# JuanDuGit/DH3D

Hardware: AMD Instinct MI355X
Metric: point-clouds/sec (higher is better)
Workload: dtype f32; 1 GPU; local-descriptor forward (basic_config), N=8192 K=8, batch=8; clouds_per_gpu=8, clouds_total=8, points=8192, knn=8, parallelism=clouds sharded over 1 GPU(s), no data-path collective, weights=random-init (no checkpoint blobs exist upstream), steps_in_flight=4

## Files before the change

### dh3d_amd/csrc/knn.hip

```cpp
#include <float.h>
#include <limits.h>

#include <type_traits>

#include "cell_walk.h"
#include "common.h"
#include "keys.h"
#include "wave_ops.h"

#pragma clang fp contract(off)

namespace {

typedef float f32x2 __attribute__((ext_vector_type(2)));
typedef unsigned long long u64;

constexpr int kQueriesPerBlock = 256;
constexpr int kChunk = 1024;
constexpr int kQueue = 16;

struct KnnLadder {
  int log2ct;
  int ctmask;
  int cv;
// ... 215 lines not shown
                                                                    int32_t *__restrict__ nn,
                                                                    float *__restrict__ dist, const int *__restrict__ gate) {
  if (gate && !gate[(size_t)blockIdx.y * kCellInts + kCellFlag]) return;
  __shared__ __attribute__((aligned(16))) float s_c[kSortedWaves][64 * 3];
  __shared__ uint2 s_q[kSortedWaves][kQueue * 64];
  __shared__ int s_id[kSortedWaves][64];
  const int b = blockIdx.y;
  const int lane = threadIdx.x & 63, wave = threadIdx.x >> 6;
  const int NG = (N + 63) / 64;
  const int g = blockIdx.x * kSortedWaves + wave;
  if (g >= NG) return;
  const float4 *sc = sorted + (size_t)b * N;
  const float4 *gb = reinterpret_cast<const float4 *>(gbox) + (size_t)b * NG * 2;
  float *my_c = s_c[wave];
  uint2 *my_q = s_q[wave];
  int *my_id = s_id[wave];

  const int qi = g * 64 + lane;
  const bool valid = qi < N;
  const float4 pad = make_float4(INFINITY, INFINITY, INFINITY, __int_as_float(-1));
  float4 qr = valid ? sc[qi] : pad;
  const f32x2 qx2 = {qr.x, qr.x}, qy2 = {qr.y, qr.y}, qz2 = {qr.z, qr.z};
  const float4 qlo = gb[g * 2], qhi = gb[g * 2 + 1];

  KnnState<KMAX> st;
#pragma unroll
  for (int i = 0; i < KMAX; ++i) st.keys[i] = ~0ull;
  st.bound = INFINITY;
  int cnt = 0;
  float wave_bound = INFINITY;

  auto drain = [&]() {
    const int deepest = -wave_min_i32(-cnt);
    uint2 nxt = my_q[lane];
#pragma unroll 1
    for (int i = 0; i < deepest; ++i) {
      const uint2 e = nxt;
      if (i + 1 < deepest) nxt = my_q[(i + 1) * 64 + lane];
      if (i < cnt) knn_offer<KMAX>(st, __uint_as_float(e.x), (int)e.y, lad);
    }
    cnt = 0;
    wave_bound = wave_max_f32(valid ? st.bound : 0.f);
  };

  auto scan_group = [&](int gcc, const float4 cr) {
    my_c[cand4_slot(lane, 0)] = cr.x;
    my_c[cand4_slot(lane, 1)] = cr.y;
    my_c[cand4_slot(lane, 2)] = cr.z;
    my_id[lane] = __float_as_int(cr.w);
    __builtin_amdgcn_wave_barrier();
    const int clen = min(64, N - gcc * 64);
    for (int j = 0; j < clen; j += 32) {
      f32x2 s[4][4];
      float mn[4];
#pragma unroll
      for (int u = 0; u < 4; ++u) {
        knn_dist8(my_c + ((j >> 2) + 2 * u) * 12, qx2, qy2, qz2, s[u]);
        mn[u] = knn_min8(s[u]);
      }
      const float m = fminf(fminf(mn[0], mn[1]), fminf(mn[2], mn[3]));
      if (__any(valid && m <= st.bound)) {
#pragma unroll
        for (int u = 0; u < 4; ++u) {
          if (valid && mn[u] <= st.bound) {
#pragma unroll
            for (int t = 0; t < 8; ++t) {
              const float sv = s[u][t >> 1][t & 1];
              if (sv <= st.bound && j + 8 * u + t < clen) {
                my_q[cnt * 64 + lane] = make_uint2(__float_as_uint(sv), (unsigned)my_id[j + 8 * u + t]);
                ++cnt;
              }
            }
          }
          if (__any(cnt > kQueue - 8)) drain();
        }
      }
    }
    __builtin_amdgcn_wave_barrier();
  };
  auto load_group = [&](int gcc) { const int ci = gcc * 64 + lane; return ci < N ? sc[ci] : pad; };

  scan_group(g, qr);
  if (__any(cnt > 0)) drain();

  const int cg = g >> 6, NC = (NG + 63) >> 6;
  for (int tier = 0; tier < 2; ++tier) {
    for (int k = 0; k < 2 * NC; ++k) {
      const int ci = cg + ((k & 1) ? (k + 1) / 2 : -(k / 2));
      if (ci < 0 || ci >= NC) continue;
      const int c0 = ci * 64, gl = min(max(g - c0, 0), 63);
      const int gi = c0 + lane;
      const bool other = gi < NG && gi != g;
      float bd = INFINITY;
      float4 clo = make_float4(INFINITY, INFINITY, INFINITY, 0.f), chi = clo;
      if (other) {
        clo = gb[gi * 2];
        chi = gb[gi * 2 + 1];
        const float ex = fmaxf(fmaxf(clo.x - qhi.x, qlo.x - chi.x), 0.f);
        const float ey = fmaxf(fmaxf(clo.y - qhi.y, qlo.y - chi.y), 0.f);
        const float ez = fmaxf(fmaxf(clo.z - qhi.z, qlo.z - chi.z), 0.f);
        bd = (ex * ex + ey * ey + ez * ez) * 0.99999f;
      }
      unsigned long long mask =
          tier == 0 ? __ballot(other && bd == 0.f) : __ballot(other && bd > 0.f && bd <= wave_bound);
      if (!mask) continue;
      int l = knn_pick_near(mask, gl);
      mask &= ~(1ull << l);
      float4 nxt = load_group(c0 + l);
      while (true) {
        const int lcur = l;
        const float4 cr = nxt;
        const bool more = mask != 0;
        if (more) {
          l = knn_pick_near(mask, gl);
          mask &= ~(1ull << l);
          nxt = load_group(c0 + l);
        }
        const float bdl = wave_bcast_f32(bd, lcur);
        if (bdl <= wave_bound) {
          const float lx = wave_bcast_f32(clo.x, lcur), ly = wave_bcast_f32(clo.y, lcur), lz = wave_bcast_f32(clo.z, lcur);
          const float hx = wave_bcast_f32(chi.x, lcur), hy = wave_bcast_f32(chi.y, lcur), hz = wave_bcast_f32(chi.z, lcur);
          const float px = fmaxf(fmaxf(lx - qr.x, qr.x - hx), 0.f);
          const float py = fmaxf(fmaxf(ly - qr.y, qr.y - hy), 0.f);
          const float pz = fmaxf(fmaxf(lz - qr.z, qr.z - hz), 0.f);
          const float pd = (px * px + py * py + pz * pz) * 0.99999f;
          if (__any(valid && pd <= st.bound)) scan_group(c0 + lcur, cr);
        }
        if (!more) break;
      }
    }
  }
  if (__any(cnt > 0)) drain();

  if (valid) {
    const int y = __float_as_int(qr.w);
    int32_t *o_nn = nn + ((size_t)b * N + y) * K;
    float *o_d = dist + ((size_t)b * N + y) * K;
#pragma unroll
    for (int i = 0; i < KMAX; ++i) {
      if (i < K) {
        const unsigned tb = (unsigned)st.keys[i];
        if (st.keys[i] == ~0ull) {
          o_nn[i] = -1;
          o_d[i] = FLT_MAX;
        } else {
          o_nn[i] = (int)(((tb % (unsigned)lad.cv) << lad.log2ct) + tb / (unsigned)lad.cv);
          o_d[i] = __uint_as_float((unsigned)(st.keys[i] >> 32));
        }
      }
    }
  }
}

template <int S>
__host__ __device__ constexpr int knn_split_lds_bytes() {
  return S * (64 * 3 * 4 + kQueue * 64 * 8 + 64 * 4 + 64 * 4 + 64 * 4);
}
template <int KMAX, int S>
__device__ __forceinline__ void knn_split_body(const float4 *__restrict__ sorted, const float *__restrict__ gbox, int N, int K,
                                               const KnnLadder lad, int32_t *__restrict__ nn, float *__restrict__ dist,
                                               const int b, const int g, unsigned char *lds, const int wave0 = 0) {
  static_assert(KMAX * 64 * sizeof(u64) <= kQueue * 64 * sizeof(uint2), "a K-list fits its wave's survivor queue");
  uint2 (*s_q)[kQueue * 64] = reinterpret_cast<uint2 (*)[kQueue * 64]>(lds);
  float (*s_c)[64 * 3] = reinterpret_cast<float (*)[64 * 3]>(lds + S * kQueue * 64 * 8);
  int (*s_id)[64] = reinterpret_cast<int (*)[64]>(lds + S * (kQueue * 64 * 8 + 64 * 3 * 4));
  float (*s_share)[64] = reinterpret_cast<float (*)[64]>(lds + S * (kQueue * 64 * 8 + 64 * 3 * 4 + 64 * 4));
  float (*s_kth)[64] = reinterpret_cast<float (*)[64]>(lds + S * (kQueue * 64 * 8 + 64 * 3 * 4 + 64 * 8));
  constexpr int R = (KMAX + S - 1) / S - 1;
  const int lane = threadIdx.x & 63;
  const int wave = __builtin_amdgcn_readfirstlane((int)(threadIdx.x >> 6) - wave0);
  const int NG = (N + 63) / 64;
  const float4 *sc = sorted + (size_t)b * N;
  const float4 *gb = reinterpret_cast<const float4 *>(gbox) + (size_t)b * NG * 2;
  float *my_c = s_c[wave];
  uint2 *my_q = s_q[wave];
  int *my_id = s_id[wave];

  const int qi = g * 64 + lane;
  const bool valid = qi < N;
  const float4 pad = make_float4(INFINITY, INFINITY, INFINITY, __int_as_float(-1));
  const float4 qr = valid ? sc[qi] : pad;
  const f32x2 qx2 = {qr.x, qr.x}, qy2 = {qr.y, qr.y}, qz2 = {qr.z, qr.z};
  const float4 qlo = gb[g * 2], qhi = gb[g * 2 + 1];

  KnnState<KMAX> st;
#pragma unroll
  for (int i = 0; i < KMAX; ++i) st.keys[i] = ~0ull;
  st.bound = INFINITY;
  int cnt = 0;
  float wave_bound = INFINITY;
  s_share[wave][lane] = INFINITY;
  s_kth[wave][lane] = INFINITY;
  __syncthreads();

  auto adopt = [&](float mx) {
    float mk = st.bound;
#pragma unroll
    for (int w = 1; w < S; ++w) {
      mx = fmaxf(mx, s_share[(wave + w) % S][lane]);
      mk = fminf(mk, s_kth[(wave + w) % S][lane]);
    }
    st.bound = fminf(mk, mx);
    wave_bound = wave_max_f32(valid ? st.bound : 0.f);
  };

  auto drain = [&]() {
    const int deepest = -wave_min_i32(-cnt);
    uint2 nxt = my_q[lane];
#pragma unroll 1
    for (int i = 0; i < deepest; ++i) {
      const uint2 e = nxt;
      if (i + 1 < deepest) nxt = my_q[(i + 1) * 64 + lane];
      if (i < cnt) knn_offer<KMAX, true>(st, __uint_as_float(e.x), (int)e.y, lad);
    }
    cnt = 0;
    const unsigned hb = (unsigned)(st.keys[R] >> 32);
    float mx = INFINITY;
    if (hb <= 0x7f800000u) {
      const float dr = __uint_as_float(hb);
      mx = __fmul_rn(__fmul_rn(dr, dr), 1.000001f);
    }
    s_share[wave][lane] = mx;
    const unsigned hk = (unsigned)(st.keys[KMAX - 1] >> 32);
    if (hk <= 0x7f800000u) {
      const float dk = __uint_as_float(hk);
      s_kth[wave][lane] = __fmul_rn(__fmul_rn(dk, dk), 1.000001f);
    }
    adopt(mx);
  };

  auto scan_group = [&](int gcc, const float4 cr) {
    my_c[cand4_slot(lane, 0)] = cr.x;
    my_c[cand4_slot(lane, 1)] = cr.y;
    my_c[cand4_slot(lane, 2)] = cr.z;
    my_id[lane] = __float_as_int(cr.w);
    __builtin_amdgcn_wave_barrier();
    const int clen = min(64, N - gcc * 64);
    for (int j = 0; j < clen; j += 32) {
      f32x2 sq[4][4];
      float mn[4];
#pragma unroll
      for (int u = 0; u < 4; ++u) {
        knn_dist8(my_c + ((j >> 2) + 2 * u) * 12, qx2, qy2, qz2, sq[u]);
        mn[u] = knn_min8(sq[u]);
      }
      const float m = fminf(fminf(mn[0], mn[1]), fminf(mn[2], mn[3]));
      if (__any(valid && m <= st.bound)) {
#pragma unroll
        for (int u = 0; u < 4; ++u) {
          if (valid && mn[u] <= st.bound) {
#pragma unroll
            for (int t = 0; t < 8; ++t) {
              const float sv = sq[u][t >> 1][t & 1];
              if (sv <= st.bound && j + 8 * u + t < clen) {
                my_q[cnt * 64 + lane] = make_uint2(__float_as_uint(sv), (unsigned)my_id[j + 8 * u + t]);
                ++cnt;
              }
            }
          }
          if (__any(cnt > kQueue - 8)) drain();
        }
      }
    }
    __builtin_amdgcn_wave_barrier();
  };
  auto load_group = [&](int gcc) { const int ci = gcc * 64 + lane; return ci < N ? sc[ci] : pad; };

  const int NO = (NG - wave + S - 1) / S, NCH = (NO + 63) >> 6;
  const int jg = g / S, cj = min(jg >> 6, max(NCH - 1, 0));
  bool other = false;
  float bd = INFINITY;
  float4 clo = make_float4(INFINITY, INFINITY, INFINITY, 0.f), chi = clo;
  auto fetch_boxes = [&](int ci) {
    const int j = ci * 64 + lane, gi = j * S + wave;
    other = j < NO && gi != g;
    if (other) {
      clo = gb[gi * 2];
      chi = gb[gi * 2 + 1];
    }
  };
  auto test_boxes = [&]() {
    bd = INFINITY;
    if (other) {
      const float ex = fmaxf(fmaxf(clo.x - qhi.x, qlo.x - chi.x), 0.f);
      const float ey = fmaxf(fmaxf(clo.y - qhi.y, qlo.y - chi.y), 0.f);
      const float ez = fmaxf(fmaxf(clo.z - qhi.z, qlo.z - chi.z), 0.f);
      bd = (ex * ex + ey * ey + ez * ez) * 0.99999f;
    }
  };
  if (NCH == 1) fetch_boxes(0);

  {
    my_c[cand4_slot(lane, 0)] = qr.x;
    my_c[cand4_slot(lane, 1)] = qr.y;
    my_c[cand4_slot(lane, 2)] = qr.z;
    my_id[lane] = __float_as_int(qr.w);
    __builtin_amdgcn_wave_barrier();
    const int clen = min(64, N - g * 64);
    for (int blk = wave; blk * 8 < clen; blk += S) {
      f32x2 sq[4];
      knn_dist8(my_c + 2 * blk * 12, qx2, qy2, qz2, sq);
      if (valid) {
#pragma unroll
        for (int t = 0; t < 8; ++t) {
          const float sv = sq[t >> 1][t & 1];
          if (sv <= st.bound && blk * 8 + t < clen) {
            my_q[cnt * 64 + lane] = make_uint2(__float_as_uint(sv), (unsigned)my_id[blk * 8 + t]);
            ++cnt;
          }
        }
      }
      if (__any(cnt > 0)) drain();
    }
    __builtin_amdgcn_wave_barrier();
    __syncthreads();
    adopt(s_share[wave][lane]);
  }
  for (int tier = 0; tier < 2; ++tier) {
    for (int k = 0; k < 2 * NCH; ++k) {
      const int ci = cj + ((k & 1) ? (k + 1) / 2 : -(k / 2));
      if (ci < 0 || ci >= NCH) continue;
      if (NCH > 1) fetch_boxes(ci);
      if (NCH > 1 || tier == 0) test_boxes();
      const int gl = min(max(jg - ci * 64, 0), 63);
      if (tier == 1) adopt(s_share[wave][lane]);
      unsigned long long mask =
          tier == 0 ? __ballot(other && bd == 0.f) : __ballot(other && bd > 0.f && bd <= wave_bound);
      if (!mask) continue;
      int l = knn_pick_near(mask, gl);
      mask &= ~(1ull << l);
      float4 nxt = load_group((ci * 64 + l) * S + wave);
      while (true) {
        const int lcur = l;
        const float4 cr = nxt;
        const bool more = mask != 0;
        if (more) {
          l = knn_pick_near(mask, gl);
          mask &= ~(1ull << l);
          nxt = load_group((ci * 64 + l) * S + wave);
        }
        const float bdl = wave_bcast_f32(bd, lcur);
        if (bdl <= wave_bound) {
          const float lx = wave_bcast_f32(clo.x, lcur), ly = wave_bcast_f32(clo.y, lcur), lz = wave_bcast_f32(clo.z, lcur);
          const float hx = wave_bcast_f32(chi.x, lcur), hy = wave_bcast_f32(chi.y, lcur), hz = wave_bcast_f32(chi.z, lcur);
          const float px = fmaxf(fmaxf(lx - qr.x, qr.x - hx), 0.f);
          const float py = fmaxf(fmaxf(ly - qr.y, qr.y - hy), 0.f);
          const float pz = fmaxf(fmaxf(lz - qr.z, qr.z - hz), 0.f);
          const float pd = (px * px + py * py + pz * pz) * 0.99999f;
          if (__any(valid && pd <= st.bound)) scan_group((ci * 64 + lcur) * S + wave, cr);
        }
        if (!more) break;
      }
    }
  }
  if (__any(cnt > 0)) drain();

  for (int step = S / 2; step >= 1; step >>= 1) {
    __syncthreads();
    if (wave >= step && wave < 2 * step) {
#pragma unroll
      for (int i = 0; i < KMAX; ++i)
        my_q[i * 64 + lane] = make_uint2((unsigned)st.keys[i], (unsigned)(st.keys[i] >> 32));
    }
    __syncthreads();
    if (wave < step) {
      const uint2 *oq = s_q[wave + step];
#pragma unroll
      for (int i = 0; i < KMAX; ++i) {
        const uint2 e = oq[i * 64 + lane];
        const u64 key = ((u64)e.y << 32) | e.x;
        if (key < st.keys[KMAX - 1]) {
          st.keys[KMAX - 1] = key;
#pragma unroll
          for (int t = KMAX - 1; t > 0; --t) {
            const u64 a = st.keys[t - 1], c = st.keys[t];
            const bool lt = c < a;
            st.keys[t - 1] = lt ? c : a;
            st.keys[t] = lt ? a : c;
          }
        }
      }
    }
  }

  if (wave == 0 && valid) {
    const int y = __float_as_int(qr.w);
    int32_t *o_nn = nn + ((size_t)b * N + y) * K;
    float *o_d = dist + ((size_t)b * N + y) * K;
#pragma unroll
    for (int i = 0; i < KMAX; ++i) {
      if (i < K) {
        const unsigned tb = (unsigned)st.keys[i];
        if (st.keys[i] == ~0ull) {
          o_nn[i] = -1;
          o_d[i] = FLT_MAX;
        } else {
          o_nn[i] = (int)(((tb % (unsigned)lad.cv) << lad.log2ct) + tb / (unsigned)lad.cv);
          o_d[i] = __uint_as_float((unsigned)(st.keys[i] >> 32));
        }
      }
    }
  }
}


template <int KMAX, int S>
__global__ __launch_bounds__(64 * S) void knn_split_kernel(const float4 *__restrict__ sorted,
                                                         const float *__restrict__ gbox, int N, int K,
                                                         KnnLadder lad, int32_t *__restrict__ nn,
                                                         float *__restrict__ dist, const int *__restrict__ gate) {
  if (gate && !gate[(size_t)blockIdx.y * kCellInts + kCellFlag]) return;
  __shared__ __attribute__((aligned(16))) unsigned char s_lds[knn_split_lds_bytes<S>()];
  const unsigned ng = (unsigned)((N + 63) / 64);
  knn_split_body<KMAX, S>(sorted, gbox, N, K, lad, nn, dist, blockIdx.y, (int)((blockIdx.x + 37u * blockIdx.y) % ng), s_lds);
}


template <int CPL>
__device__ __forceinline__ void knn_small_select_all(float (&s)[CPL], int N, int K, const KnnLadder &lad, int lane,
                                                     unsigned &my_hi, unsigned &my_lo) {
  int ln = lane;
  asm volatile("" : "+v"(ln));
  unsigned kd[CPL];
#pragma unroll
  for (int c = 0; c < CPL; ++c) kd[c] = ln + 64 * c < N ? __float_as_uint(sqrtf(s[c])) : 0xFFFFFFFFu;
  u64 need = 0;
  u64 m1 = ~0ull, m2 = ~0ull;
  bool more = false;
  auto rescan = [&]() {
    m1 = ~0ull; m2 = ~0ull;
    int cnt = 0;
    asm volatile("" : "+v"(ln));
#pragma unroll
    for (int c = 0; c < CPL; ++c) {
      const int j = ln + 64 * c;
      const unsigned tb = j < N ? (unsigned)((j & lad.ctmask) * lad.cv + (j >> lad.log2ct)) : 0xFFFFFFFFu;
      const u64 key = ((u64)kd[c] << 32) | tb;
      const bool ok = key >= need && key != ~0ull;
      const bool c1 = ok && key < m1, c2 = ok && key < m2;
      m2 = c1 ? m1 : (c2 ? key : m2);
      m1 = c1 ? key : m1;
      cnt += ok ? 1 : 0;
    }
    more = cnt > 2;
  };
  rescan();
  for (int r = 0; r < K; ++r) {
    const unsigned hi = wave_min_u32((unsigned)(m1 >> 32));
    const unsigned lo = wave_min_u32((unsigned)(m1 >> 32) == hi ? (unsigned)m1 : 0xFFFFFFFFu);
    if (lane == r) { my_hi = hi; my_lo = lo; }
    const u64 sel = ((u64)hi << 32) | lo;
    if (sel == ~0ull) break;
    need = sel + 1;
    const bool won = m1 == sel;
    const bool dry = won && m2 == ~0ull && more;
    m1 = won ? m2 : m1;
    m2 = won ? ~0ull : m2;
    if (__ballot(dry) != 0ull) rescan();
  }
}
// ... 120 lines not shown
    return dh3d_launch_status();                                                                                 \
  }
    DH3D_SMALL_CASE(8) DH3D_SMALL_CASE(16) DH3D_SMALL_CASE(32)
#undef DH3D_SMALL_CASE
    return DH3D_ERR_UNSUPPORTED;
  }
  dim3 grid(dh3d_cdiv(N, kQueriesPerBlock), B), block(kQueriesPerBlock);
#define DH3D_LANE_CASE(KM)                                                                                       \
  if (p.kmax == KM) {                                                                                            \
    hipLaunchKernelGGL((knn_kernel<KM, XYZ>), grid, block, 0, s, pos, N, K, lad, nn, dist);                      \
    return dh3d_launch_status();                                                                                 \
  }
  DH3D_LANE_CASE(4) DH3D_LANE_CASE(8) DH3D_LANE_CASE(16) DH3D_LANE_CASE(32) DH3D_LANE_CASE(64)
#undef DH3D_LANE_CASE
  return DH3D_ERR_UNSUPPORTED;
}

template <int KMAX>
__global__ __launch_bounds__(256) void knn_anydp_kernel(const float *__restrict__ pos, int Dp, int N, int K, KnnLadder lad,
                                                        int32_t *__restrict__ nn, float *__restrict__ dist) {
  __shared__ float s_c[16][256];
  const int b = blockIdx.y, y = blockIdx.x * 256 + threadIdx.x;
  const float *pc = pos + (size_t)b * Dp * N;
  float q[16];
#pragma unroll
  for (int dp = 0; dp < 16; ++dp) q[dp] = (dp < Dp && y < N) ? pc[(size_t)dp * N + y] : 0.f;
  u64 keys[KMAX];
#pragma unroll
  for (int i = 0; i < KMAX; ++i) keys[i] = ~0ull;
  for (int x0 = 0; x0 < N; x0 += 256) {
    __syncthreads();
    for (int dp = 0; dp < Dp; ++dp) s_c[dp][threadIdx.x] = x0 + (int)threadIdx.x < N ? pc[(size_t)dp * N + x0 + threadIdx.x] : 0.f;
    __syncthreads();
    const int cnt = min(256, N - x0);
    for (int j = 0; j < cnt; ++j) {
      float sum = 0.f;
      for (int dp = 0; dp < Dp; ++dp) {
        const float val = s_c[dp][j] - q[dp];
        sum = __builtin_fmaf(val, val, sum);
      }
      const float d = sqrtf(sum);
      const int x = x0 + j;
      const unsigned tb = (unsigned)((x & lad.ctmask) * lad.cv + (x >> lad.log2ct));
      const u64 key = ((u64)__float_as_uint(d) << 32) | tb;
      if (key < keys[K - 1]) {
        int i = K - 1;
        while (i > 0 && keys[i - 1] > key) { keys[i] = keys[i - 1]; --i; }
        keys[i] = key;
      }
    }
  }
  if (y >= N) return;
  int32_t *o_nn = nn + ((size_t)b * N + y) * K;
  float *o_d = dist + ((size_t)b * N + y) * K;
  for (int i = 0; i < K; ++i) {
    if (keys[i] == ~0ull) { o_nn[i] = -1; o_d[i] = 3.402823466e+38f; continue; }
    const unsigned tb = (unsigned)keys[i];
    o_nn[i] = (int)(((tb % (unsigned)lad.cv) << lad.log2ct) + tb / (unsigned)lad.cv);
    o_d[i] = __uint_as_float((unsigned)(keys[i] >> 32));
  }
}

}

DH3D_API int dh3d_knn_bruteforce(const float *positions, int B, int Dp, int N, int K, int32_t *nn,
                                 float *dist, void *stream) {
  DH3D_REQUIRE(positions && nn && dist && B > 0 && N > 0 && K > 0 && Dp > 0);
  DH3D_SUPPORTED(K <= kKnnMaxK && B <= kKnnMaxB);
  if (Dp == 3) return knn_launch<false>(positions, B, N, K, nn, dist, (hipStream_t)stream);
  DH3D_SUPPORTED(Dp <= kAnyDpMax);
  const KnnLadder lad = knn_ladder(N);
  dim3 grid(dh3d_cdiv(N, 256), B), block(256);
  hipStream_t s = (hipStream_t)stream;
  const int km = knn_anydp_width(K);
#define DH3D_ANYDP_CASE(KM)                                                                                      \
  if (km == KM) {                                                                                                \
    hipLaunchKernelGGL(knn_anydp_kernel<KM>, grid, block, 0, s, positions, Dp, N, K, lad, nn, dist);             \
    return dh3d_launch_status();                                                                                 \
  }
  DH3D_ANYDP_CASE(8) DH3D_ANYDP_CASE(16) DH3D_ANYDP_CASE(64)
#undef DH3D_ANYDP_CASE
  return DH3D_ERR_UNSUPPORTED;
}

DH3D_API int dh3d_knn_bruteforce_xyz(const float *xyz, int B, int N, int K, int32_t *nn, float *dist,
                                     void *stream) {
  DH3D_REQUIRE(xyz && nn && dist && B > 0 && N > 0 && K > 0);
  DH3D_SUPPORTED(K <= kKnnMaxK && B <= kKnnMaxB);
  return knn_launch<true>(xyz, B, N, K, nn, dist, (hipStream_t)stream);
}

DH3D_API int dh3d_knn_bruteforce_plan(int B, int Dp, int N, int K) {
  if (!(B > 0 && N > 0 && K > 0 && Dp > 0) || !(K <= kKnnMaxK && B <= kKnnMaxB)) return -1;
  if (Dp != 3) return Dp <= kAnyDpMax ? 3 * 65536 + knn_anydp_width(K) : -1;
  const KnnPlan p = knn_plan(B, N, K);
  return p.cpl > 0 ? 1 * 65536 + p.cpl * 256 + p.q : 2 * 65536 + p.kmax;
}

struct KnnSortedPlan {
  int s, kmax;
};
static KnnSortedPlan knn_sorted_plan(int B, int N, int K) {
  const long long groups = (long long)((N + 63) / 64) * B;
  KnnSortedPlan p{groups <= 256 ? 8 : groups <= 1280 ? 4 : groups <= 4096 ? 2 : 0, knn_list_width(K)};
  if (p.kmax > 16) p.s = 0;
  if (p.s == 8 && p.kmax == 4) p.kmax = 8;
  return p;
}

static int knn_sorted_launch(const float *sorted, const float *gbox, int B, int N, int K, int32_t *nn, float *dist,
                             const int *gate, void *stream) {
  DH3D_REQUIRE(sorted && gbox && nn && dist && B > 0 && N > 0 && K > 0);
  DH3D_SUPPORTED(K <= kKnnMaxK && B <= kKnnMaxB);
  const KnnLadder lad = knn_ladder(N);
  const int NG = (N + 63) / 64;
  dim3 grid(dh3d_cdiv(NG, kSortedWaves), B), block(64 * kSortedWaves);
  hipStream_t s = (hipStream_t)stream;
  const float4 *so = reinterpret_cast<const float4 *>(sorted);
  const KnnSortedPlan p = knn_sorted_plan(B, N, K);
  if (p.s > 0) {
    dim3 sgrid(NG, B);
#define DH3D_SPLIT_CASE(KM, SS)                                                                               \
  if (p.kmax == KM && p.s == SS) {                                                                           \
    hipLaunchKernelGGL((knn_split_kernel<KM, SS>), sgrid, dim3(64 * SS), 0, s, so, gbox, N, K, lad, nn, dist, gate); \
    return dh3d_launch_status();                                                                             \
  }
    DH3D_SPLIT_CASE(4, 2) DH3D_SPLIT_CASE(4, 4)
    DH3D_SPLIT_CASE(8, 2) DH3D_SPLIT_CASE(8, 4) DH3D_SPLIT_CASE(8, 8)
    DH3D_SPLIT_CASE(16, 2) DH3D_SPLIT_CASE(16, 4) DH3D_SPLIT_CASE(16, 8)
#undef DH3D_SPLIT_CASE
    return DH3D_ERR_UNSUPPORTED;
  }
#define DH3D_SORTED_CASE(KM)                                                                                  \
  if (p.kmax == KM) {                                                                                        \
    hipLaunchKernelGGL((knn_sorted_kernel<KM>), grid, block, 0, s, so, gbox, N, K, lad, nn, dist, gate);      \
    return dh3d_launch_status();                                                                             \
  }
  DH3D_SORTED_CASE(4) DH3D_SORTED_CASE(8) DH3D_SORTED_CASE(16) DH3D_SORTED_CASE(32) DH3D_SORTED_CASE(64)
#undef DH3D_SORTED_CASE
  return DH3D_ERR_UNSUPPORTED;
}

DH3D_API int dh3d_knn_sorted(const float *sorted, const float *gbox, int B, int N, int K, int32_t *nn,
                             float *dist, void *stream) {
  return knn_sorted_launch(sorted, gbox, B, N, K, nn, dist, nullptr, stream);
}

DH3D_API int dh3d_knn_sorted_plan(int B, int N, int K) {
  if (!(B > 0 && N > 0 && K > 0) || !(K <= kKnnMaxK && B <= kKnnMaxB)) return -1;
  const KnnSortedPlan p = knn_sorted_plan(B, N, K);
  return p.s * 256 + p.kmax;
}

constexpr int kGridCap = 256;
constexpr int kGridRow = kGridCap + 2;
constexpr int kGridScreenCap = 80;
static_assert(kGridScreenCap % 16 == 0 && kGridScreenCap * 6 <= kGridCap * 2, "the screened drain's row");

__device__ __forceinline__ unsigned knn_spread4(unsigned v) {
  return (v & 1u) | ((v & 2u) << 2) | ((v & 4u) << 4) | ((v & 8u) << 6);
}
__device__ __forceinline__ void knn_cswap(u64 &a, u64 &b) {
  const bool lt = b < a;
  const u64 lo = lt ? b : a, hi = lt ? a : b;
  a = lo; b = hi;
}
template <int CTRL>
__device__ __forceinline__ u64 knn_dpp_u64(u64 v) {
  const int lo = __builtin_amdgcn_update_dpp(0, (int)(unsigned)v, CTRL, 0xF, 0xF, true);
  const int hi = __builtin_amdgcn_update_dpp(0, (int)(unsigned)(v >> 32), CTRL, 0xF, 0xF, true);
  return ((u64)(unsigned)hi << 32) | (unsigned)lo;
}
template <int CTRL>
__device__ __forceinline__ int knn_dpp_i32(int v) {
  return __builtin_amdgcn_update_dpp(0, v, CTRL, 0xF, 0xF, true);
}
template <int CTRL>
__device__ __forceinline__ void knn_merge_step(KnnState<8> &st) {
  u64 c[8];
#pragma unroll
  for (int i = 0; i < 8; ++i) {
    const u64 mine = st.keys[i], theirs = knn_dpp_u64<CTRL>(st.keys[7 - i]);
    c[i] = mine < theirs ? mine : theirs;
  }
  knn_cswap(c[0], c[4]); knn_cswap(c[1], c[5]); knn_cswap(c[2], c[6]); knn_cswap(c[3], c[7]);
  knn_cswap(c[0], c[2]); knn_cswap(c[1], c[3]); knn_cswap(c[4], c[6]); knn_cswap(c[5], c[7]);
  knn_cswap(c[0], c[1]); knn_cswap(c[2], c[3]); knn_cswap(c[4], c[5]); knn_cswap(c[6], c[7]);
#pragma unroll
  for (int i = 0; i < 8; ++i) st.keys[i] = c[i];
}
__device__ __forceinline__ void knn_bound_of_list(KnnState<8> &st) {
  const unsigned hb = (unsigned)(st.keys[7] >> 32);
  if (hb <= 0x7f800000u) {
    const float dk = __uint_as_float(hb);
    st.bound = __fmul_rn(__fmul_rn(dk, dk), 1.000001f);
  }
}
template <int L>
__device__ __forceinline__ void knn_merge_sublanes(KnnState<8> &st) {
  if (L >= 2) knn_merge_step<0xB1>(st);
  if (L >= 4) knn_merge_step<0x4E>(st);
  if (L >= 8) knn_merge_step<0x141>(st);
  knn_bound_of_list(st);
}
template <int L>
__device__ __forceinline__ void knn_merge_after_sparse_pass(KnnState<8> &st, int sub) {
  if (L != 4 || __any(sub != 0 && st.keys[0] != ~0ull)) {
    knn_merge_sublanes<L>(st);
    return;
  }
#pragma unroll
  for (int i = 0; i < 8; ++i) st.keys[i] = knn_dpp_u64<0x00>(st.keys[i]);
  knn_bound_of_list(st);
}

template <int L, int SF>
__global__ __launch_bounds__(256) void knn_grid_kernel(const float4 *__restrict__ sorted, const float *__restrict__ gbox,
                                                      const int *__restrict__ cells, int N, int K, int D, KnnLadder lad,
                                                      int32_t *__restrict__ nn, float *__restrict__ dist) {
  constexpr int QB = 256 / L;
  static_assert(SF == 0 || (L == 4 && SF <= 4), "the merged scan: 64 queries per workgroup, at most four waves");
  constexpr int kGridLds = 3 * 64 * 4 + QB * kGridRow * 2 + QB * 4;
  constexpr int kSplitLds = SF == 2 ? 2 * knn_split_lds_bytes<2>() : SF > 0 ? knn_split_lds_bytes<(SF > 0 ? SF : 1)>() : 0;
  __shared__ __attribute__((aligned(16))) unsigned char s_raw[kGridLds > kSplitLds ? kGridLds : kSplitLds];
  const int b = blockIdx.y, lane = threadIdx.x & 63, sub = lane & (L - 1);
  if (cells[(size_t)b * kCellInts + kCellFlag]) {
    if constexpr (SF > 0) {
      const int ngq = (N + 63) / 64;
      if constexpr (SF == 2) {
        const int half = (int)(threadIdx.x >> 7), pairs = (ngq + 1) / 2;
        if ((int)blockIdx.x >= pairs) return;
        const int g0 = (int)blockIdx.x + half * pairs;
        if (g0 >= ngq) return;
        knn_split_body<8, 2>(sorted, gbox, N, K, lad, nn, dist, b, (int)(((unsigned)g0 + 37u * (unsigned)b) % (unsigned)ngq),
                             s_raw + half * knn_split_lds_bytes<2>(), half * 2);
      } else if (threadIdx.x < 64 * SF) {
        knn_split_body<8, (SF > 0 ? SF : 1)>(sorted, gbox, N, K, lad, nn, dist, b, (int)((blockIdx.x + 37u * (unsigned)b) % (unsigned)ngq), s_raw);
      }
    }
    return;
  }
  const int qi = (int)((blockIdx.x + 37u * (unsigned)b) % gridDim.x) * QB + threadIdx.x / L;
  const bool valid = qi < N;
  const float4 *sc = sorted + (size_t)b * N;
  const CellGrid g = cell_grid(cells, b);
  const int *ct = g.ct;
  const float lo[3] = {g.lo[0], g.lo[1], g.lo[2]}, scl[3] = {g.scl[0], g.scl[1], g.scl[2]};
  const int nb[3] = {g.nb[0], g.nb[1], g.nb[2]};
  const float4 qr = sc[valid ? qi : N - 1];
  const float q[3] = {qr.x, qr.y, qr.z};
  int nc[3], drop[3];
  sched_bits(g.sched, nc, kGridSteps - D);
#pragma unroll
  for (int a = 0; a < 3; ++a) drop[a] = nb[a] - nc[a];
  const int span = 1 << D;
  int cq[3], gmax[3];
  float w[3], eps[3];
#pragma unroll
  for (int a = 0; a < 3; ++a) {
    cq[a] = min((4 << nb[a]) - 1, max(0, (int)((q[a] - lo[a]) * scl[a]))) >> (2 + drop[a]);
    gmax[a] = ((1 << nb[a]) >> drop[a]) - 1;
    w[a] = (float)(4 << drop[a]) / scl[a];
    eps[a] = 2.5e-6f * ((float)(4 << nb[a]) / scl[a]);
  }
  unsigned (*s_ctab)[64] = reinterpret_cast<unsigned (*)[64]>(s_raw);
  cell_deposit_tables(g.sched, nc[0], nc[1], nc[2], kGridSteps - D, s_ctab);
  auto tab_code = [&](int ax, int ay, int az) { return s_ctab[0][ax & 63] | s_ctab[1][ay & 63] | s_ctab[2][az & 63]; };
  KnnState<8> st;
#pragma unroll
  for (int i = 0; i < 8; ++i) st.keys[i] = ~0ull;
  st.bound = valid ? INFINITY : -1.f;

  auto axis_d2 = [&](int a, int o) {
    const float l = lo[a] + (float)(cq[a] + o) * w[a];
    const float d = fmaxf(fmaxf(fmaxf(l - q[a], q[a] - (l + w[a])), 0.f) - eps[a], 0.f);
    return d * d;
  };
  float d2x[5];
  unsigned bitx[5];
  bool okx[5];
#pragma unroll
  for (int t = 0; t < 5; ++t) {
    const int ax = cq[0] + t - 2;
    okx[t] = (unsigned)ax <= (unsigned)gmax[0];
    d2x[t] = okx[t] ? axis_d2(0, t - 2) : INFINITY;
    bitx[t] = s_ctab[0][ax & 63];
  }
  auto inside = [&](int R) {
    float G = INFINITY;
#pragma unroll
    for (int a = 0; a < 3; ++a) {
      if (cq[a] - R > 0) G = fminf(G, (q[a] - (lo[a] + (float)(cq[a] - R) * w[a])) - eps[a]);
      if (cq[a] + R < gmax[a]) G = fminf(G, ((lo[a] + (float)(cq[a] + R + 1) * w[a]) - q[a]) - eps[a]);
    }
    if (G == INFINITY) return true;
    G = fmaxf(G, 0.f);
    return st.bound < G * G * 0.99999f;
  };

  auto keep_one_copy = [&]() {
    if (sub != 0) {
#pragma unroll
      for (int i = 0; i < 8; ++i) st.keys[i] = ~0ull;
    }
  };
  unsigned short (*s_list)[kGridRow] = reinterpret_cast<unsigned short (*)[kGridRow]>(s_raw + 3 * 64 * 4);
  int *s_cnt = reinterpret_cast<int *>(s_raw + 3 * 64 * 4 + QB * kGridRow * 2);
  const int qs = threadIdx.x / L;
  auto direct = [&](int j) {
    const float4 r = sc[j];
    const float dx = r.x - q[0], dy = r.y - q[1], dz = r.z - q[2];
    knn_offer<8, false>(st, fmaf(dz, dz, fmaf(dy, dy, dx * dx)), __float_as_int(r.w), lad);
  };
  auto enqueue = [&](int beg, int end) {
    const int len = end - beg;
    if (len <= 0) return;
    const int off = atomicAdd(&s_cnt[qs], len);
    const int fit = min(len, kGridCap - off);
    for (int k = 0; k < fit; ++k) s_list[qs][off + k] = (unsigned short)(beg + k);
    for (int k = max(fit, 0); k < len; ++k) direct(beg + k);
  };
  auto drain_screened = [&]() __attribute__((always_inline)) {
    const int T = s_cnt[qs];
    if constexpr (L != 4) return min(T, kGridCap);
    const bool screen = !__any(T > kGridScreenCap) && __any(T > 32);
    const int ns = screen ? T : 0;
    unsigned short *row = s_list[qs];
    float *s2v = reinterpret_cast<float *>(row + kGridScreenCap);
    float m1 = INFINITY, m2 = INFINITY;
#pragma unroll 1
    for (int k0 = 0; k0 < ns; k0 += 4 * L) {
      float4 r[4];
#pragma unroll
      for (int u = 0; u < 4; ++u) r[u] = sc[row[min(k0 + sub + u * L, ns - 1)]];
      wave_lds_sync();
#pragma unroll
      for (int u = 0; u < 4; ++u) {
        const int i = k0 + sub + u * L;
        const float dx = r[u].x - q[0], dy = r[u].y - q[1], dz = r[u].z - q[2];
        const float s = i < ns ? fmaf(dz, dz, fmaf(dy, dy, dx * dx)) : __builtin_nanf("");
        m2 = s < m1 ? m1 : fminf(m2, s);
        m1 = fminf(m1, s);
        s2v[i] = s;
        row[i] = (unsigned short)__float_as_int(r[u].w);
      }
    }
    float U = m2;
    U = fmaxf(U, __int_as_float(knn_dpp_i32<0xB1>(__float_as_int(U))));
    U = fmaxf(U, __int_as_float(knn_dpp_i32<0x4E>(__float_as_int(U))));
    const float thr = __fmul_rn(U, 1.000001f);
    wave_lds_sync();
    int c = 0;
#pragma unroll 1
    for (int k0 = 0; k0 < ns; k0 += 4 * L) {
      float s[4];
      unsigned short id[4];
#pragma unroll
      for (int u = 0; u < 4; ++u) {
        s[u] = s2v[k0 + sub + u * L];
        id[u] = row[k0 + sub + u * L];
      }
      wave_lds_sync();
      int n = 0, at[4];
#pragma unroll
      for (int u = 0; u < 4; ++u) {
        at[u] = n;
        n += s[u] <= thr ? 1 : 0;
      }
      const int n1 = knn_dpp_i32<0x90>(n);
      int p = n + (sub >= 1 ? n1 : 0);
      const int p2 = knn_dpp_i32<0x40>(p);
      p += sub >= 2 ? p2 : 0;
      const int first = c + p - n;
#pragma unroll
      for (int u = 0; u < 4; ++u)
        if (s[u] <= thr) {
          s2v[first + at[u]] = s[u];
          row[first + at[u]] = id[u];
        }
      c += knn_dpp_i32<0xFF>(p);
      wave_lds_sync();
    }
    float s_n = s2v[sub];
    int id_n = row[sub];
#pragma unroll 1
    for (int j = sub; j < c; j += L) {
      const float s = s_n;
      const int id = id_n;
      const int jn = min(j + L, kGridScreenCap - 1);
      s_n = s2v[jn];
      id_n = row[jn];
      knn_offer<8, false>(st, s, id, lad);
    }
    return screen ? 0 : min(T, kGridCap);
  };
  auto drain = [&](auto screen) __attribute__((always_inline)) {
    wave_lds_sync();
    int total;
    if constexpr (decltype(screen)::value) total = drain_screened();
    else total = min(s_cnt[qs], kGridCap);
#pragma unroll 1
    for (int base = sub; base < total; base += 4 * L) {
      float4 r[4];
      bool ok[4];
#pragma unroll
      for (int u = 0; u < 4; ++u) {
        const int i = base + u * L;
        ok[u] = i < total;
        r[u] = sc[s_list[qs][min(i, total - 1)]];
      }
#pragma unroll
      for (int u = 0; u < 4; ++u) {
        const float dx = r[u].x - q[0], dy = r[u].y - q[1], dz = r[u].z - q[2];
        const float s2 = fmaf(dz, dz, fmaf(dy, dy, dx * dx));
        knn_offer<8, false>(st, ok[u] ? s2 : __builtin_nanf(""), __float_as_int(r[u].w), lad);
      }
    }
    wave_lds_sync();
  };
  auto column = [&](auto tmask, int dy, int dz) __attribute__((always_inline)) {
    constexpr int TMASK = decltype(tmask)::value;
    const int ay = cq[1] + dy - 2, az = cq[2] + dz - 2;
    if ((unsigned)ay > (unsigned)gmax[1] || (unsigned)az > (unsigned)gmax[2]) return;
    const float d2yz = axis_d2(1, dy - 2) + axis_d2(2, dz - 2);
    const unsigned bityz = tab_code(0, ay, az);
    int beg[5], end[5];
#pragma unroll
    for (int t = 0; t < 5; ++t)
      if (TMASK >> t & 1) {
        beg[t] = ct[bityz | bitx[t]];
        end[t] = ct[(bityz | bitx[t]) + span];
      }
    if constexpr (TMASK != 0b01110) {
#pragma unroll
      for (int t = 0; t < 5; ++t)
        if (TMASK >> t & 1) {
          if (!okx[t] || (d2yz + d2x[t]) * 0.99999f > st.bound) continue;
          enqueue(beg[t], end[t]);
        }
    } else {
      int len[5], tot = 0;
#pragma unroll
      for (int t = 0; t < 5; ++t)
        if (TMASK >> t & 1) {
          len[t] = okx[t] && !((d2yz + d2x[t]) * 0.99999f > st.bound) ? end[t] - beg[t] : 0;
          tot += len[t];
        }
      if (tot == 0) return;
      int off = atomicAdd(&s_cnt[qs], tot);
#pragma unroll
      for (int t = 0; t < 5; ++t)
        if (TMASK >> t & 1) {
          const int fit = min(len[t], kGridCap - off);
          unsigned short *dst = &s_list[qs][off];
#pragma unroll
          for (int k = 0; k < 4; ++k)
            if (k < fit) dst[k] = (unsigned short)(beg[t] + k);
          for (int k = 4; k < fit; ++k) dst[k] = (unsigned short)(beg[t] + k);
          for (int k = max(fit, 0); k < len[t]; ++k) direct(beg[t] + k);
          off += len[t];
        }
    }
  };
  auto begin_pass = [&]() __attribute__((always_inline)) {
    if (sub == 0) s_cnt[qs] = 0;
    __builtin_amdgcn_fence(__ATOMIC_SEQ_CST, "wavefront");
    __builtin_amdgcn_wave_barrier();
  };
  begin_pass();
  if constexpr (L == 4) {
    const int ay = cq[1] + 1, az = cq[2] + 1;
    const bool mine = sub < 3 && (unsigned)ay <= (unsigned)gmax[1] && (unsigned)az <= (unsigned)gmax[2];
    const bool okc = sub == 0 ? okx[1] : sub == 1 ? okx[2] : okx[3];
    const float d2c = (sub == 0 ? d2x[1] : sub == 1 ? d2x[2] : d2x[3]) + axis_d2(1, 1) + axis_d2(2, 1);
    const unsigned code = tab_code(0, ay, az) | (sub == 0 ? bitx[1] : sub == 1 ? bitx[2] : bitx[3]);
    const int beg9 = ct[mine ? code : 0], end9 = ct[mine ? code + span : 0];
#pragma unroll 1
    for (int ci = sub; ci < 8; ci += L) column(std::integral_constant<int, 0b01110>{}, 1 + ci % 3, 1 + ci / 3);
    if (mine && okc && !(d2c * 0.99999f > st.bound)) enqueue(beg9, end9);
  } else {
#pragma unroll 1
    for (int ci = sub; ci < 9; ci += L) column(std::integral_constant<int, 0b01110>{}, 1 + ci % 3, 1 + ci / 3);
  }
  drain(std::true_type{});
  knn_merge_sublanes<L>(st);
  keep_one_copy();
  begin_pass();
  bool exact = false;
  int ylo = -2, zlo = -2, ny = 5, ncol = valid ? 25 : 0;
  if (valid && st.bound < INFINITY) {
    const float r = sqrtf(st.bound) * 1.0001f;
    int dlo[3], dhi[3];
#pragma unroll
    for (int a = 0; a < 3; ++a) {
      const float inv = scl[a] / (float)(4 << drop[a]);
      dlo[a] = min(0, max(0, (int)floorf((q[a] - r - eps[a] - lo[a]) * inv)) - cq[a]);
      dhi[a] = max(0, min(gmax[a], (int)floorf((q[a] + r + eps[a] - lo[a]) * inv)) - cq[a]);
    }
    const int by = dhi[1] - dlo[1] + 1, bc = by * (dhi[2] - dlo[2] + 1);
    if (dlo[0] >= -2 && dhi[0] <= 2 && bc <= 128) {
      exact = true;
      ylo = dlo[1]; zlo = dlo[2]; ny = by; ncol = bc;
    }
  }
#pragma unroll 1
  for (int ci = sub; ci < ncol; ci += L) {
    const int iz = ci / ny, dy = ylo + (ci - iz * ny), dz = zlo + iz;
    if (abs(dy) <= 1 && abs(dz) <= 1) column(std::integral_constant<int, 0b10001>{}, dy + 2, dz + 2);
    else column(std::integral_constant<int, 0b11111>{}, dy + 2, dz + 2);
  }
  drain(std::false_type{});
  knn_merge_after_sparse_pass<L>(st, sub);
  const bool done = !valid || exact || inside(2);
  if (__any(!done)) {
    if (done) {
      keep_one_copy();
    } else {
#pragma unroll
      for (int i = 0; i < 8; ++i) st.keys[i] = ~0ull;
      const int NG = (N + 63) >> 6;
      const float4 *gb = reinterpret_cast<const float4 *>(gbox) + (size_t)b * NG * 2;
#pragma unroll 1
      for (int g = sub; g < NG; g += L) {
        const float4 lo4 = gb[2 * g], hi4 = gb[2 * g + 1];
        const float ex = fmaxf(fmaxf(lo4.x - q[0], q[0] - hi4.x), 0.f), ey = fmaxf(fmaxf(lo4.y - q[1], q[1] - hi4.y), 0.f),
                    ez = fmaxf(fmaxf(lo4.z - q[2], q[2] - hi4.z), 0.f);
        if ((ex * ex + ey * ey + ez * ez) * 0.99999f > st.bound) continue;
        const int j1 = min(N, g * 64 + 64);
#pragma unroll 1
        for (int j = g * 64; j < j1; j += 8) {
          float4 r8[8];
#pragma unroll
          for (int u = 0; u < 8; ++u) r8[u] = sc[min(j + u, j1 - 1)];
#pragma unroll
          for (int u = 0; u < 8; ++u) {
            const float dx = r8[u].x - q[0], dy = r8[u].y - q[1], dz = r8[u].z - q[2];
            const float s2 = fmaf(dz, dz, fmaf(dy, dy, dx * dx));
            knn_offer<8, false>(st, j + u < j1 ? s2 : __builtin_nanf(""), __float_as_int(r8[u].w), lad);
          }
        }
      }
    }
    knn_merge_sublanes<L>(st);
  }
  if (valid) {
    const int y = __float_as_int(qr.w);
#pragma unroll
    for (int e = 0; e < 8 / L; ++e) {
      const int slot = e * L + sub;
      if (slot >= K) break;
      u64 key = st.keys[0];
#pragma unroll
      for (int i = 1; i < 8; ++i) key = slot == i ? st.keys[i] : key;
      const size_t o = ((size_t)b * N + y) * K + slot;
      if (key == ~0ull) {
        nn[o] = -1;
        dist[o] = FLT_MAX;
      } else {
        const unsigned tb = (unsigned)key;
        nn[o] = (int)(((tb % (unsigned)lad.cv) << lad.log2ct) + tb / (unsigned)lad.cv);
        dist[o] = __uint_as_float((unsigned)(key >> 32));
      }
    }
  }
}

constexpr int kGridLanes = 4;

struct KnnGridPlan {
  int sf, drop;
};
static KnnGridPlan knn_grid_plan(int B, int N) {
  KnnGridPlan p{0, 0};
  while (p.drop < 6 && ((long long)N << p.drop) <= 3072) ++p.drop;
  const long long groups = (long long)((N + 63) / 64) * B;
  if (kGridLanes == 4 && groups <= 4096) p.sf = groups > 1280 ? 2 : 4;
  return p;
}

DH3D_API int dh3d_knn_grid_plan(int B, int N, int K) {
  if (B <= 0 || N <= 0 || K <= 0 || K > 8 || N > 16384 || B > 65535) return -1;
  const KnnGridPlan p = knn_grid_plan(B, N);
  return p.sf + 16 * p.drop;
}

DH3D_API int dh3d_knn_grid(const float *sorted, const float *gbox, const int32_t *cells, int B, int N, int K, int32_t *nn,
                           float *dist, void *stream) {
  DH3D_REQUIRE(sorted && gbox && cells && nn && dist && B > 0 && N > 0 && K > 0);
  DH3D_SUPPORTED(K <= 8 && N <= 16384 && B <= 65535);
  const KnnLadder lad = knn_ladder(N);
  constexpr int kLanes = kGridLanes;
  const KnnGridPlan plan = knn_grid_plan(B, N);
  const int D = plan.drop;
  const dim3 grid(dh3d_cdiv(N, 256 / kLanes), B);
  const float4 *so = reinterpret_cast<const float4 *>(sorted);
  if (plan.sf == 2) {
    hipLaunchKernelGGL((knn_grid_kernel<4, 2>), grid, dim3(256), 0, (hipStream_t)stream, so, gbox, cells, N, K, D, lad, nn, dist);
    return dh3d_launch_status();
  }
  if (plan.sf == 4) {
    hipLaunchKernelGGL((knn_grid_kernel<4, 4>), grid, dim3(256), 0, (hipStream_t)stream, so, gbox, cells, N, K, D, lad, nn, dist);
    return dh3d_launch_status();
  }
  hipLaunchKernelGGL((knn_grid_kernel<kLanes, 0>), grid, dim3(256), 0, (hipStream_t)stream, so, gbox, cells, N, K, D, lad, nn, dist);
  if (dh3d_launch_status() != DH3D_OK) return DH3D_ERR_LAUNCH;
  return knn_sorted_launch(sorted, gbox, B, N, K, nn, dist, cells, stream);
}
```

Baseline: 41260 point-clouds/sec.

## Slim KNN LDS and registers to fit five workgroups per CU

Adds a SLIM variant of the split-scan survivor queue that stores distances as floats and ids as 16-bit shorts instead of 8-byte pairs, and halves the scan unroll for that variant. It also shrinks the grid list capacity so the per-row stride is an odd number of dwords, and asserts the merged kernel fits in 32 KB of LDS so five workgroups can reside per CU. Register pressure is cut by packing the per-column x-bits and ok flags into scalars, hoisting a uniform inverse scale via readfirstlane, and disabling vectorisation of the short fill loops. The risks are 16-bit ids capping the point count, less ILP from the smaller unroll, and overflow to the slower direct path now that the list capacity is smaller.

```diff
diff --git a/dh3d_amd/csrc/knn.hip b/dh3d_amd/csrc/knn.hip
--- a/dh3d_amd/csrc/knn.hip
+++ b/dh3d_amd/csrc/knn.hip
@@ -391,20 +391,22 @@
   }
 }
 
-template <int S>
+template <int S, bool SLIM = false>
 __host__ __device__ constexpr int knn_split_lds_bytes() {
-  return S * (64 * 3 * 4 + kQueue * 64 * 8 + 64 * 4 + 64 * 4 + 64 * 4);
-}
-template <int KMAX, int S>
+  return S * (64 * 3 * 4 + kQueue * 64 * (SLIM ? 6 : 8) + 64 * 4 + 64 * 4 + 64 * 4);
+}
+template <int KMAX, int S, bool SLIM = false>
 __device__ __forceinline__ void knn_split_body(const float4 *__restrict__ sorted, const float *__restrict__ gbox, int N, int K,
                                                const KnnLadder lad, int32_t *__restrict__ nn, float *__restrict__ dist,
                                                const int b, const int g, unsigned char *lds, const int wave0 = 0) {
-  static_assert(KMAX * 64 * sizeof(u64) <= kQueue * 64 * sizeof(uint2), "a K-list fits its wave's survivor queue");
-  uint2 (*s_q)[kQueue * 64] = reinterpret_cast<uint2 (*)[kQueue * 64]>(lds);
-  float (*s_c)[64 * 3] = reinterpret_cast<float (*)[64 * 3]>(lds + S * kQueue * 64 * 8);
-  int (*s_id)[64] = reinterpret_cast<int (*)[64]>(lds + S * (kQueue * 64 * 8 + 64 * 3 * 4));
-  float (*s_share)[64] = reinterpret_cast<float (*)[64]>(lds + S * (kQueue * 64 * 8 + 64 * 3 * 4 + 64 * 4));
-  float (*s_kth)[64] = reinterpret_cast<float (*)[64]>(lds + S * (kQueue * 64 * 8 + 64 * 3 * 4 + 64 * 8));
+  constexpr int kQBytes = kQueue * 64 * (SLIM ? 6 : 8);
+  constexpr int U = SLIM ? 2 : 4;
+  static_assert(KMAX * 64 * sizeof(u64) <= kQBytes && kQBytes % 16 == 0, "a K-list fits its wave's survivor queue");
+  uint2 (*s_q)[kQBytes / 8] = reinterpret_cast<uint2 (*)[kQBytes / 8]>(lds);
+  float (*s_c)[64 * 3] = reinterpret_cast<float (*)[64 * 3]>(lds + S * kQBytes);
+  int (*s_id)[64] = reinterpret_cast<int (*)[64]>(lds + S * (kQBytes + 64 * 3 * 4));
+  float (*s_share)[64] = reinterpret_cast<float (*)[64]>(lds + S * (kQBytes + 64 * 3 * 4 + 64 * 4));
+  float (*s_kth)[64] = reinterpret_cast<float (*)[64]>(lds + S * (kQBytes + 64 * 3 * 4 + 64 * 8));
   constexpr int R = (KMAX + S - 1) / S - 1;
   const int lane = threadIdx.x & 63;
   const int wave = __builtin_amdgcn_readfirstlane((int)(threadIdx.x >> 6) - wave0);
@@ -414,6 +416,20 @@
   float *my_c = s_c[wave];
   uint2 *my_q = s_q[wave];
   int *my_id = s_id[wave];
+  float *my_qs = reinterpret_cast<float *>(my_q);
+  unsigned short *my_qid = reinterpret_cast<unsigned short *>(my_qs + kQueue * 64);
+  auto q_put = [&](int slot, float sv, int id) {
+    if constexpr (SLIM) {
+      my_qs[slot * 64 + lane] = sv;
+      my_qid[slot * 64 + lane] = (unsigned short)id;
+    } else {
+      my_q[slot * 64 + lane] = make_uint2(__float_as_uint(sv), (unsigned)id);
+    }
+  };
+  auto q_get = [&](int slot) {
+    if constexpr (SLIM) return make_uint2(__float_as_uint(my_qs[slot * 64 + lane]), (unsigned)my_qid[slot * 64 + lane]);
+    else return my_q[slot * 64 + lane];
+  };
 
   const int qi = g * 64 + lane;
   const bool valid = qi < N;
@@ -445,11 +461,11 @@
 
   auto drain = [&]() {
     const int deepest = -wave_min_i32(-cnt);
-    uint2 nxt = my_q[lane];
+    uint2 nxt = q_get(0);
 #pragma unroll 1
     for (int i = 0; i < deepest; ++i) {
       const uint2 e = nxt;
-      if (i + 1 < deepest) nxt = my_q[(i + 1) * 64 + lane];
+      if (i + 1 < deepest) nxt = q_get(i + 1);
       if (i < cnt) knn_offer<KMAX, true>(st, __uint_as_float(e.x), (int)e.y, lad);
     }
     cnt = 0;
@@ -475,24 +491,25 @@
     my_id[lane] = __float_as_int(cr.w);
     __builtin_amdgcn_wave_barrier();
     const int clen = min(64, N - gcc * 64);
-    for (int j = 0; j < clen; j += 32) {
-      f32x2 sq[4][4];
-      float mn[4];
-#pragma unroll
-      for (int u = 0; u < 4; ++u) {
+    for (int j = 0; j < clen; j += 8 * U) {
+      f32x2 sq[U][4];
+      float mn[U];
+#pragma unroll
+      for (int u = 0; u < U; ++u) {
         knn_dist8(my_c + ((j >> 2) + 2 * u) * 12, qx2, qy2, qz2, sq[u]);
         mn[u] = knn_min8(sq[u]);
       }
-      const float m = fminf(fminf(mn[0], mn[1]), fminf(mn[2], mn[3]));
+      float m = fminf(mn[0], mn[1]);
+      if constexpr (U == 4) m = fminf(m, fminf(mn[2], mn[3]));
       if (__any(valid && m <= st.bound)) {
 #pragma unroll
-        for (int u = 0; u < 4; ++u) {
+        for (int u = 0; u < U; ++u) {
           if (valid && mn[u] <= st.bound) {
 #pragma unroll
             for (int t = 0; t < 8; ++t) {
               const float sv = sq[u][t >> 1][t & 1];
               if (sv <= st.bound && j + 8 * u + t < clen) {
-                my_q[cnt * 64 + lane] = make_uint2(__float_as_uint(sv), (unsigned)my_id[j + 8 * u + t]);
+                q_put(cnt, sv, my_id[j + 8 * u + t]);
                 ++cnt;
               }
             }
@@ -544,7 +561,7 @@
         for (int t = 0; t < 8; ++t) {
           const float sv = sq[t >> 1][t & 1];
           if (sv <= st.bound && blk * 8 + t < clen) {
-            my_q[cnt * 64 + lane] = make_uint2(__float_as_uint(sv), (unsigned)my_id[blk * 8 + t]);
+            q_put(cnt, sv, my_id[blk * 8 + t]);
             ++cnt;
           }
         }
@@ -971,10 +988,12 @@
   return p.s * 256 + p.kmax;
 }
 
-constexpr int kGridCap = 256;
+constexpr int kGridCap = 240;
 constexpr int kGridRow = kGridCap + 2;
+static_assert(kGridRow % 2 == 0 && (kGridRow / 2) % 2 == 1, "a row is an odd number of dwords");
 constexpr int kGridScreenCap = 80;
 static_assert(kGridScreenCap % 16 == 0 && kGridScreenCap * 6 <= kGridCap * 2, "the screened drain's row");
+static_assert(knn_split_lds_bytes<4, true>() <= 32768, "the aliased scan block");
 
 __device__ __forceinline__ unsigned knn_spread4(unsigned v) {
   return (v & 1u) | ((v & 2u) << 2) | ((v & 4u) << 4) | ((v & 8u) << 6);
@@ -1014,6 +1033,9 @@
     const float dk = __uint_as_float(hb);
     st.bound = __fmul_rn(__fmul_rn(dk, dk), 1.000001f);
   }
+}
+__device__ __forceinline__ float knn_uniform_f32(float v) {
+  return __int_as_float(__builtin_amdgcn_readfirstlane(__float_as_int(v)));
 }
 template <int L>
 __device__ __forceinline__ void knn_merge_sublanes(KnnState<8> &st) {
@@ -1040,8 +1062,9 @@
   constexpr int QB = 256 / L;
   static_assert(SF == 0 || (L == 4 && SF <= 4), "the merged scan: 64 queries per workgroup, at most four waves");
   constexpr int kGridLds = 3 * 64 * 4 + QB * kGridRow * 2 + QB * 4;
-  constexpr int kSplitLds = SF == 2 ? 2 * knn_split_lds_bytes<2>() : SF > 0 ? knn_split_lds_bytes<(SF > 0 ? SF : 1)>() : 0;
+  constexpr int kSplitLds = SF == 2 ? 2 * knn_split_lds_bytes<2>() : SF > 0 ? knn_split_lds_bytes<(SF > 0 ? SF : 1), SF == 4>() : 0;
   __shared__ __attribute__((aligned(16))) unsigned char s_raw[kGridLds > kSplitLds ? kGridLds : kSplitLds];
+  static_assert(SF != 4 || sizeof(s_raw) <= 32768, "knn_grid_kernel<4, 4>: five workgroups per CU");
   const int b = blockIdx.y, lane = threadIdx.x & 63, sub = lane & (L - 1);
   if (cells[(size_t)b * kCellInts + kCellFlag]) {
     if constexpr (SF > 0) {
@@ -1054,7 +1077,7 @@
         knn_split_body<8, 2>(sorted, gbox, N, K, lad, nn, dist, b, (int)(((unsigned)g0 + 37u * (unsigned)b) % (unsigned)ngq),
                              s_raw + half * knn_split_lds_bytes<2>(), half * 2);
       } else if (threadIdx.x < 64 * SF) {
-        knn_split_body<8, (SF > 0 ? SF : 1)>(sorted, gbox, N, K, lad, nn, dist, b, (int)((blockIdx.x + 37u * (unsigned)b) % (unsigned)ngq), s_raw);
+        knn_split_body<8, (SF > 0 ? SF : 1), SF == 4>(sorted, gbox, N, K, lad, nn, dist, b, (int)((blockIdx.x + 37u * (unsigned)b) % (unsigned)ngq), s_raw);
       }
     }
     return;
@@ -1074,13 +1097,14 @@
   for (int a = 0; a < 3; ++a) drop[a] = nb[a] - nc[a];
   const int span = 1 << D;
   int cq[3], gmax[3];
-  float w[3], eps[3];
+  float w[3], eps[3], inv[3];
 #pragma unroll
   for (int a = 0; a < 3; ++a) {
     cq[a] = min((4 << nb[a]) - 1, max(0, (int)((q[a] - lo[a]) * scl[a]))) >> (2 + drop[a]);
     gmax[a] = ((1 << nb[a]) >> drop[a]) - 1;
-    w[a] = (float)(4 << drop[a]) / scl[a];
-    eps[a] = 2.5e-6f * ((float)(4 << nb[a]) / scl[a]);
+    w[a] = knn_uniform_f32((float)(4 << drop[a]) / scl[a]);
+    eps[a] = knn_uniform_f32(2.5e-6f * ((float)(4 << nb[a]) / scl[a]));
+    inv[a] = knn_uniform_f32(scl[a] / (float)(4 << drop[a]));
   }
   unsigned (*s_ctab)[64] = reinterpret_cast<unsigned (*)[64]>(s_raw);
   cell_deposit_tables(g.sched, nc[0], nc[1], nc[2], kGridSteps - D, s_ctab);
@@ -1096,15 +1120,18 @@
     return d * d;
   };
   float d2x[5];
-  unsigned bitx[5];
-  bool okx[5];
+  u64 bitx_all = 0;
+  unsigned okx_all = 0;
 #pragma unroll
   for (int t = 0; t < 5; ++t) {
     const int ax = cq[0] + t - 2;
-    okx[t] = (unsigned)ax <= (unsigned)gmax[0];
-    d2x[t] = okx[t] ? axis_d2(0, t - 2) : INFINITY;
-    bitx[t] = s_ctab[0][ax & 63];
-  }
+    const bool ok = (unsigned)ax <= (unsigned)gmax[0];
+    okx_all |= ok ? 1u << t : 0u;
+    d2x[t] = ok ? axis_d2(0, t - 2) : INFINITY;
+    bitx_all |= (u64)s_ctab[0][ax & 63] << (12 * t);
+  }
+  auto bitx = [&](int t) { return (unsigned)(bitx_all >> (12 * t)) & 0xFFFu; };
+  auto okx = [&](int t) { return (okx_all >> t & 1u) != 0; };
   auto inside = [&](int R) {
     float G = INFINITY;
 #pragma unroll
@@ -1136,6 +1163,7 @@
     if (len <= 0) return;
     const int off = atomicAdd(&s_cnt[qs], len);
     const int fit = min(len, kGridCap - off);
+#pragma clang loop vectorize(disable) unroll(disable)
     for (int k = 0; k < fit; ++k) s_list[qs][off + k] = (unsigned short)(beg + k);
     for (int k = max(fit, 0); k < len; ++k) direct(beg + k);
   };
@@ -1247,14 +1275,14 @@
 #pragma unroll
     for (int t = 0; t < 5; ++t)
       if (TMASK >> t & 1) {
-        beg[t] = ct[bityz | bitx[t]];
-        end[t] = ct[(bityz | bitx[t]) + span];
+        beg[t] = ct[bityz | bitx(t)];
+        end[t] = ct[(bityz | bitx(t)) + span];
       }
     if constexpr (TMASK != 0b01110) {
 #pragma unroll
       for (int t = 0; t < 5; ++t)
         if (TMASK >> t & 1) {
-          if (!okx[t] || (d2yz + d2x[t]) * 0.99999f > st.bound) continue;
+          if (!okx(t) || (d2yz + d2x[t]) * 0.99999f > st.bound) continue;
           enqueue(beg[t], end[t]);
         }
     } else {
@@ -1262,7 +1290,7 @@
 #pragma unroll
       for (int t = 0; t < 5; ++t)
         if (TMASK >> t & 1) {
-          len[t] = okx[t] && !((d2yz + d2x[t]) * 0.99999f > st.bound) ? end[t] - beg[t] : 0;
+          len[t] = okx(t) && !((d2yz + d2x[t]) * 0.99999f > st.bound) ? end[t] - beg[t] : 0;
           tot += len[t];
         }
       if (tot == 0) return;
@@ -1275,6 +1303,7 @@
 #pragma unroll
           for (int k = 0; k < 4; ++k)
             if (k < fit) dst[k] = (unsigned short)(beg[t] + k);
+#pragma clang loop vectorize(disable) unroll(disable)
           for (int k = 4; k < fit; ++k) dst[k] = (unsigned short)(beg[t] + k);
           for (int k = max(fit, 0); k < len[t]; ++k) direct(beg[t] + k);
           off += len[t];
@@ -1290,9 +1319,9 @@
   if constexpr (L == 4) {
     const int ay = cq[1] + 1, az = cq[2] + 1;
     const bool mine = sub < 3 && (unsigned)ay <= (unsigned)gmax[1] && (unsigned)az <= (unsigned)gmax[2];
-    const bool okc = sub == 0 ? okx[1] : sub == 1 ? okx[2] : okx[3];
+    const bool okc = sub == 0 ? okx(1) : sub == 1 ? okx(2) : okx(3);
     const float d2c = (sub == 0 ? d2x[1] : sub == 1 ? d2x[2] : d2x[3]) + axis_d2(1, 1) + axis_d2(2, 1);
-    const unsigned code = tab_code(0, ay, az) | (sub == 0 ? bitx[1] : sub == 1 ? bitx[2] : bitx[3]);
+    const unsigned code = tab_code(0, ay, az) | (sub == 0 ? bitx(1) : sub == 1 ? bitx(2) : bitx(3));
     const int beg9 = ct[mine ? code : 0], end9 = ct[mine ? code + span : 0];
 #pragma unroll 1
     for (int ci = sub; ci < 8; ci += L) column(std::integral_constant<int, 0b01110>{}, 1 + ci % 3, 1 + ci / 3);
@@ -1312,9 +1341,8 @@
     int dlo[3], dhi[3];
 #pragma unroll
     for (int a = 0; a < 3; ++a) {
-      const float inv = scl[a] / (float)(4 << drop[a]);
-      dlo[a] = min(0, max(0, (int)floorf((q[a] - r - eps[a] - lo[a]) * inv)) - cq[a]);
-      dhi[a] = max(0, min(gmax[a], (int)floorf((q[a] + r + eps[a] - lo[a]) * inv)) - cq[a]);
+      dlo[a] = min(0, max(0, (int)floorf((q[a] - r - eps[a] - lo[a]) * inv[a])) - cq[a]);
+      dhi[a] = max(0, min(gmax[a], (int)floorf((q[a] + r + eps[a] - lo[a]) * inv[a])) - cq[a]);
     }
     const int by = dhi[1] - dlo[1] + 1, bc = by * (dhi[2] - dlo[2] + 1);
     if (dlo[0] >= -2 && dhi[0] <= 2 && bc <= 128) {
```

Result: no change. 41790 point-clouds/sec (median of 2 runs) (+1.3%).
